# zhoujoey/ORB-SLAM3-Mac

Hardware: AMD Instinct MI355X
Metric: ORB extract+match frames/sec (higher is better)
Workload: dtype u8; 1 GPU; vga: synthetic 640x480 batch=1024 per GPU, 8-level pyramid, 1000 feats/frame, ORB extract + Hamming 2-NN match (Frame.cc:1146) + SearchForInitialization (ORBmatcher.cc:710) vs successor frame; pipelines=1, matchers=side by side (two contexts), frames_total=1024

## Files before the change

### include/orbhip.h

```cpp
#ifndef ORBHIP_H
#define ORBHIP_H
#include <stddef.h>
#include <stdint.h>
#ifdef __cplusplus
extern "C" {
#endif

#define ORBHIP_OK 0
#define ORBHIP_E_BADARG (-1)
#define ORBHIP_E_NODEVICE (-2)
#define ORBHIP_E_HIP (-3)
#define ORBHIP_E_CAPACITY (-4)
#define ORBHIP_E_ABORTED (-5)
#define ORBHIP_E_NOTSPD (-6)
#define ORBHIP_E_EMPTY (-7)

typedef struct {
    float x, y, size, angle, response;
    int32_t octave, class_id;
} orbhip_keypoint;

typedef struct orbhip_ctx orbhip_ctx;
typedef struct orbhip_extractor orbhip_extractor;

// ... 26 lines not shown
int orbhip_extractor_results(orbhip_extractor *ext, orbhip_keypoint **d_kp, uint8_t **d_desc,
                             int32_t **d_count, int32_t **d_mono_index);
int orbhip_extract_batch_host(orbhip_extractor *ext, const uint8_t *h_images, int width, int height,
                              size_t row_stride, size_t frame_stride, int batch, int lap0, int lap1,
                              orbhip_keypoint *kp_out, uint8_t *desc_out, int cap,
                              int32_t *count_out, int32_t *mono_out);
int orbhip_extract_batch_host_view(orbhip_extractor *ext, const uint8_t *h_images, int width, int height, size_t row_stride,
                                   size_t frame_stride, int batch, int lap0, int lap1, const orbhip_keypoint **kp_view,
                                   const uint8_t **desc_view, int *row_capacity, const int32_t **count_view, const int32_t **mono_view);
int orbhip_extractor_blur_kernel(const orbhip_extractor *ext, int batch);
int orbhip_extractor_fast_kernel(const orbhip_extractor *ext);
int orbhip_extractor_blur_tiled(const orbhip_extractor *ext, int batch);
int orbhip_extractor_desc_plan(const orbhip_extractor *ext, int batch, int32_t *kp_base, int32_t *kp_cap, int32_t *waves_per_xcd);

int orbhip_extractor_resize_band_rows(const orbhip_extractor *ext, int level);

int orbhip_extractor_last_frame(orbhip_extractor *ext, int frame, const orbhip_keypoint **d_kp, const uint8_t **d_desc,
                                const orbhip_keypoint **h_kp_view, const uint8_t **h_desc_view, int32_t *count, unsigned long long *generation);

int orbhip_extractor_level_dims(const orbhip_extractor *ext, int level, int *w, int *h);
int orbhip_extractor_get_pyramid_level(orbhip_extractor *ext, int frame, int level, int padded,
                                       uint8_t *h_out, size_t out_stride);
int orbhip_extractor_get_pyramid_padded(orbhip_extractor *ext, int frame, uint8_t *const *levels_out, const size_t *strides);
int orbhip_extractor_get_blurred_level(orbhip_extractor *ext, int frame, int level,
                                       uint8_t *h_out, size_t out_stride);
int orbhip_extractor_get_fast_candidates(orbhip_extractor *ext, int frame, int level,
                                         int32_t *xs, int32_t *ys, int32_t *scores, int cap,
                                         int32_t *n_out);
int orbhip_extractor_get_level_keypoints(orbhip_extractor *ext, int frame, int level,
                                         orbhip_keypoint *out, int cap, int32_t *n_out);
// ... 612 lines not shown
```

### orb-slam3-mac_amd/csrc/orb_internal.h

```cpp
#pragma once
#include <hip/hip_runtime.h>
#include <stdint.h>
#include <vector>
#include "../../include/orbhip.h"

#define ORB_MAX_LEVELS 16
#define ORB_EDGE 19
#define ORB_MINB 16
#define ORB_HALF_PATCH 15
#define ORB_RS_STEPS 24

struct OrbLevel {
    uint8_t *img;
    uint8_t *blur;
    size_t img_frame_stride;
    size_t blur_frame_stride;
    int w, h, img_pitch, blur_pitch;
    int blur_tiles_x;
    int ncols, nrows, wcell, hcell;
    int cell_base;
    int cell_cap;
    int quota;
    int key_base, key_cap;
    int kp_base, kp_cap;
// ... 102 lines not shown
    const int32_t *nL, *nR;
    float mb, mbf;
    float *u_right, *depth;
    int32_t *sad, *n_kept;
};
void orb_launch_stereo(const StereoArgs &A, hipStream_t s);

int orb_lds_optin(const void *func, int device, size_t need);

void orb_plan_fast(const OrbParams &P, FastParams &F);
bool orb_plan_resize(OrbParams &P, int level, const std::vector<int16_t> &xofs, const std::vector<int16_t> &xalpha, const std::vector<int16_t> &yofs,
                     const std::vector<int16_t> &ybeta, std::vector<uint32_t> &xchunk, std::vector<uint32_t> &ytab);
bool orb_plan_blur(OrbParams &P, std::vector<int8_t> &bm_th, std::vector<int8_t> &bm_tv);
int orb_blur_kernel(const OrbParams &P, int batch);

void orb_launch_resize(const OrbParams &P, int level, hipStream_t s);
void orb_launch_fast_cells(const FastParams &F, hipStream_t s, int max_per_cu, int lvl_lo = 0, int lvl_hi = -1);
const void *orb_fast_runs_func(int nld);
int orb_fast_runs_nld(const FastParams &F);
int orb_fast_variant(const FastParams &F);
const void *orb_fast_cells_func(int small);
#define ORB_OVERLAP_MIN_BATCH 16
#ifndef BLR_R
#define BLR_R 24
#endif
void orb_launch_blur(const OrbParams &P, hipStream_t s, int wgs_per_cu, int frame0 = 0, int nframes = -1);
void orb_launch_orient_desc(const OrbParams &P, hipStream_t s);
int orb_orient_desc_blocks(const OrbParams &P);
void orb_launch_octree(const OrbParams &P, hipStream_t s, int parts = 3);
void orb_launch_assemble(const OrbParams &P, hipStream_t s);
size_t orb_octree_lds_bytes(int nc);
// ... 4 lines not shown
```

### orb-slam3-mac_amd/csrc/orbhip_api.hip

```cpp
#include "orb_internal.h"
#include "ctx_internal.h"
#include <cmath>
#include <cfloat>
#include <cstdio>
#include <cstdlib>
#include <cstring>
#include <string>
#include <vector>
#include <mutex>
#include <set>
#include <utility>

static thread_local std::string g_last_error;
extern "C" const char *orbhip_last_error(void) { return g_last_error.c_str(); }
extern "C" const char *orbhip_version(void) { return "orbhip 0.1 (gfx950)"; }

#define HIP_TRY(expr)                                                                   \
    do {                                                                                \
        hipError_t _e = (expr);                                                         \
        if (_e != hipSuccess) {                                                         \
            g_last_error = std::string(#expr) + ": " + hipGetErrorString(_e);           \
            return ORBHIP_E_HIP;                                                        \
        }                                                                               \
    } while (0)
// ... 189 lines not shown
static inline int align_up(int v, int a) { return (v + a - 1) / a * a; }

#define ORBHIP_PROF_SLOTS 32
struct orbhip_extractor {
    orbhip_ctx *ctx;
    int nfeatures, nlevels, ini_th, min_th;
    float scale_factor;
    float scale[ORB_MAX_LEVELS], inv_scale[ORB_MAX_LEVELS], sigma2[ORB_MAX_LEVELS], inv_sigma2[ORB_MAX_LEVELS];
    int per_level[ORB_MAX_LEVELS];
    int umax[ORB_HALF_PATCH + 1];
    int gauss_q8[7];
    int width, height, max_batch;
    bool level0_owned;
    OrbParams P;
    FastParams F;
    std::vector<void *> allocs;
    size_t bytes_reserved;
    int last_batch;
    bool profiling;
    hipEvent_t ev[ORBHIP_PROF_SLOTS][ORBHIP_STAGE_COUNT + 1];
    int ev_calls;
    bool ev_created;
    float stage_ms[ORBHIP_STAGE_COUNT];
    uint8_t *d_level0;
    int32_t *d_stereo_sad;
    bool graph_mode, graph_valid;
    hipStream_t aux; hipEvent_t ev_fork, ev_join, ev_pyr; bool aux_ok; int overlap;
    hipGraphExec_t graph_exec;
    int g_w, g_h, g_batch, g_lap0, g_lap1;
    size_t level0_frame_stride; int level0_pitch;
// ... 96 lines not shown
extern "C" int orbhip_extractor_max_keypoints(const orbhip_extractor *e) { return e ? e->P.max_kp : ORBHIP_E_BADARG; }

template <typename T>
static int dev_alloc(orbhip_extractor *e, T **p, size_t count)
{
    void *q = nullptr;
    size_t bytes = std::max<size_t>(count * sizeof(T), 256);
    hipError_t err = hipMalloc(&q, bytes);
    if (err != hipSuccess) { g_last_error = std::string("hipMalloc: ") + hipGetErrorString(err); return ORBHIP_E_HIP; }
    e->allocs.push_back(q);
    e->bytes_reserved += bytes;
    *p = (T *)q;
    return ORBHIP_OK;
}

static void resize_tables(int sn, int dn, bool horizontal, std::vector<int16_t> &ofs, std::vector<int16_t> &coef)
{
    double scale = 1. / ((double)dn / sn);
    ofs.resize(dn); coef.resize(2 * dn);
    for (int d = 0; d < dn; d++) {
        float f = (float)((d + 0.5) * scale - 0.5);
        int s = (int)floorf(f);
        f -= s;
        if (horizontal) {
            if (s < 0) { f = 0; s = 0; }
            if (s >= sn - 1) { f = 0; s = sn - 1; }
        }
        int c0 = cv_round_f((1.f - f) * 2048), c1 = cv_round_f(f * 2048);
        ofs[d] = (int16_t)std::min(std::max(s, -32768), 32767);
        coef[2 * d] = (int16_t)std::min(std::max(c0, -32768), 32767);
        coef[2 * d + 1] = (int16_t)std::min(std::max(c1, -32768), 32767);
    }
}

extern "C" int orbhip_blur_half_widths(int *out19)
{
    if (!out19) return ORBHIP_E_BADARG;
    static const int8_t pat[1024] = {
#include "orb_pattern.inc"
    };
    double R2 = 0;
    for (int i = 0; i < 512; i++) R2 = std::max(R2, (double)pat[2 * i] * pat[2 * i] + (double)pat[2 * i + 1] * pat[2 * i + 1]);
    for (int d = 0; d < ORB_EDGE; d++) {
        const double t = std::max(d - 0.5, 0.0), q = R2 - t * t;
        out19[d] = q > 0 ? std::min((int)floor(sqrt(q) + 0.5), 18) : -64;
    }
    return ORBHIP_OK;
}

// ... 35 lines not shown
        OrbLevel &L = P.lv[l];
        L.cell_cap = max_cell_cap;
        L.key_base = keys;
        L.key_cap = std::min(L.ncols * L.nrows * max_cell_cap, ((L.w - 2 * ORB_MINB + 1) / 2 + L.ncols) * ((L.h - 2 * ORB_MINB + 1) / 2 + L.nrows));
        L.key_cap = std::min(L.key_cap, 0xFFFFF);
        keys += align_up(L.key_cap, 4);
    }
    P.cells_per_frame = cells; P.keys_per_frame = keys; P.kps_per_frame = kps; P.max_kp = align_up(kps, 8);
    orb_plan_fast(P, e->F);
    P.rows_min_batch = getenv("ORBHIP_ROWS_MIN_BATCH") ? atoi(getenv("ORBHIP_ROWS_MIN_BATCH")) : 16;
    std::vector<int8_t> bm_th, bm_tv;
    const bool bm_ok = orb_plan_blur(P, bm_th, bm_tv);
    P.cell_list_frame_stride = (size_t)cells * max_cell_cap;
    int rc;
    const size_t B = (size_t)max_batch;
    for (int l = 0; l < e->nlevels; l++) {
        OrbLevel &L = P.lv[l];
        L.img_pitch = align_up(L.w, 64); L.blur_pitch = L.img_pitch;
        L.img_frame_stride = (size_t)L.img_pitch * L.h;
        L.blur_tiles_x = (L.w + 15) / 16;
        L.blur_frame_stride = align_up(std::max((size_t)L.blur_pitch * L.h, (size_t)L.blur_tiles_x * ((L.h + 7) / 8) * 128), (size_t)128);
        if ((rc = dev_alloc(e, &L.img, B * L.img_frame_stride + 64))) return rc;
        if ((rc = dev_alloc(e, &L.blur, B * L.blur_frame_stride + 64))) return rc;
        if (l > 0) {
            std::vector<int16_t> xo, xa, yo, yb;
            resize_tables(P.lv[l - 1].w, L.w, true, xo, xa);
            resize_tables(P.lv[l - 1].h, L.h, false, yo, yb);
            int16_t *dxo, *dxa, *dyo, *dyb;
            if ((rc = dev_alloc(e, &dxo, xo.size()))) return rc;
            if ((rc = dev_alloc(e, &dxa, xa.size()))) return rc;
            if ((rc = dev_alloc(e, &dyo, yo.size()))) return rc;
            if ((rc = dev_alloc(e, &dyb, yb.size()))) return rc;
            HIP_TRY(hipMemcpy(dxo, xo.data(), xo.size() * 2, hipMemcpyHostToDevice));
            HIP_TRY(hipMemcpy(dxa, xa.data(), xa.size() * 2, hipMemcpyHostToDevice));
            HIP_TRY(hipMemcpy(dyo, yo.data(), yo.size() * 2, hipMemcpyHostToDevice));
            HIP_TRY(hipMemcpy(dyb, yb.data(), yb.size() * 2, hipMemcpyHostToDevice));
            L.xofs = dxo; L.xalpha = dxa; L.yofs = dyo; L.ybeta = dyb;
            L.xchunk = nullptr; L.ytab = nullptr;
            std::vector<uint32_t> xc, yt;
            if (orb_plan_resize(P, l, xo, xa, yo, yb, xc, yt)) {
                uint32_t *dxc, *dyt;
                if ((rc = dev_alloc(e, &dxc, xc.size()))) return rc;
                if ((rc = dev_alloc(e, &dyt, yt.size()))) return rc;
                HIP_TRY(hipMemcpy(dxc, xc.data(), xc.size() * 4, hipMemcpyHostToDevice));
                HIP_TRY(hipMemcpy(dyt, yt.data(), yt.size() * 4, hipMemcpyHostToDevice));
                L.xchunk = dxc; L.ytab = dyt;
            }
        }
    }
    e->d_level0 = P.lv[0].img; e->level0_pitch = P.lv[0].img_pitch; e->level0_frame_stride = P.lv[0].img_frame_stride;
    if (bm_ok) {
        uint4 *dth, *dtv;
        if ((rc = dev_alloc(e, &dth, bm_th.size() / 16))) return rc;
        if ((rc = dev_alloc(e, &dtv, bm_tv.size() / 16))) return rc;
        HIP_TRY(hipMemcpy(dth, bm_th.data(), bm_th.size(), hipMemcpyHostToDevice));
        HIP_TRY(hipMemcpy(dtv, bm_tv.data(), bm_tv.size(), hipMemcpyHostToDevice));
        P.bm_th = dth; P.bm_tv = dtv;
    }
    P.desc_blocks_cap = getenv("ORBHIP_TUNE_DESC_BLOCKS") ? atoi(getenv("ORBHIP_TUNE_DESC_BLOCKS")) : 0;
    orbhip_blur_half_widths(P.blur_hw);
    if ((rc = dev_alloc(e, &P.cell_count, B * cells))) return rc;
// ... 181 lines not shown
    return orb_fast_variant(e->F);
}

extern "C" int orbhip_extractor_blur_tiled(const orbhip_extractor *e, int batch)
{
    if (!e || !e->max_batch) return -1;
    return e->P.blur_tiled_ok && orb_blur_kernel(e->P, batch) == 2 ? 1 : 0;
}

extern "C" int orbhip_extractor_resize_band_rows(const orbhip_extractor *e, int level)
{
    if (!e || !e->max_batch || level < 1 || level >= e->nlevels) return -1;
    return e->P.lv[level].xchunk ? e->P.lv[level].rs_rows : 0;
}

extern "C" int orbhip_extractor_set_profiling(orbhip_extractor *e, int enable)
{
    if (!e) return ORBHIP_E_BADARG;
    if (enable && !e->ev_created) {
        for (auto &slot : e->ev) for (auto &ev : slot) HIP_TRY(hipEventCreate(&ev));
        e->ev_created = true;
    }
    e->profiling = enable != 0;
    e->ev_calls = 0;
    return ORBHIP_OK;
}

extern "C" int orbhip_extractor_stage_ms(orbhip_extractor *e, float *ms_out)
{
    if (!e || !ms_out || !e->ev_created || e->ev_calls <= 0) return ORBHIP_E_BADARG;
// ... 29 lines not shown
        HIP_TRY(hipEventCreateWithFlags(&e->ev_fork, hipEventDisableTiming));
        HIP_TRY(hipEventCreateWithFlags(&e->ev_join, hipEventDisableTiming));
        HIP_TRY(hipEventCreateWithFlags(&e->ev_pyr, hipEventDisableTiming));
        e->aux_ok = true;
    }
    FastParams &F = e->F;
    for (int l = 0; l < e->nlevels; l++) { F.lv[l].img = P.lv[l].img; F.lv[l].frame_stride = P.lv[l].img_frame_stride; F.lv[l].img_pitch = P.lv[l].img_pitch; }
    F.batch = batch; F.n_cus = e->ctx->n_cus; F.cell_count = P.cell_count; F.cell_list = P.cell_list; F.cell_list_frame_stride = P.cell_list_frame_stride; F.status = P.status;
    const bool rows = orb_blur_kernel(P, batch) != 0;
    const int fast_waves = fork ? tune_int("ORBHIP_TUNE_FAST_WAVES", rows ? 18 : 10) : 0;
    STAGE_MARK(ORBHIP_STAGE_PYRAMID);
    if (fork && e->nlevels > 1 && rows && tune_int("ORBHIP_TUNE_L0_EARLY", 0)) {
        HIP_TRY(hipEventRecord(e->ev_fork, s));
        HIP_TRY(hipStreamWaitEvent(e->aux, e->ev_fork, 0));
        orb_launch_fast_cells(F, s, fast_waves, 0, 1);
        for (int l = 1; l < e->nlevels; l++) orb_launch_resize(P, l, e->aux);
        HIP_TRY(hipEventRecord(e->ev_pyr, e->aux));
        HIP_TRY(hipStreamWaitEvent(s, e->ev_pyr, 0));
        orb_launch_fast_cells(F, s, fast_waves, 1, e->nlevels);
        orb_launch_blur(P, e->aux, 5);
        HIP_TRY(hipEventRecord(e->ev_join, e->aux));
    } else {
        for (int l = 1; l < e->nlevels; l++) orb_launch_resize(P, l, s);
        STAGE_MARK(ORBHIP_STAGE_FAST_CELLS);
        if (fork) {
            HIP_TRY(hipEventRecord(e->ev_fork, s));
            HIP_TRY(hipStreamWaitEvent(e->aux, e->ev_fork, 0));
        }
        orb_launch_fast_cells(F, s, fast_waves);
        if (fork) {
            if (!tune_int("ORBHIP_TUNE_SKIP_BLUR", 0))
                orb_launch_blur(P, e->aux, tune_int("ORBHIP_TUNE_BLUR_WGS", 5));
            HIP_TRY(hipEventRecord(e->ev_join, e->aux));
        }
    }
    STAGE_MARK(ORBHIP_STAGE_BLUR);
    if (!fork) orb_launch_blur(P, s, 8);
    STAGE_MARK(ORBHIP_STAGE_OCTREE);
// ... 385 lines not shown
```

### orb-slam3-mac_amd/csrc/pyramid_kernels.hip

```cpp
#include "orb_internal.h"
#include "wave_dpp.h"
#include <algorithm>
#include <cstdlib>

#define RS_TW 64
#define RS_TH 32
#define RS_MAXC 144
#define RS_MAXR 68
__global__ __launch_bounds__(256) void k_resize(OrbParams P, int level)
{
    __shared__ __attribute__((aligned(16))) uint32_t in[RS_MAXR * (RS_MAXC / 4)];
    __shared__ uint16_t hz[RS_MAXR * RS_TW];
    const OrbLevel &D = P.lv[level];
    const OrbLevel &S = P.lv[level - 1];
    const int tid = threadIdx.x;
    const int ntx = (D.w + RS_TW - 1) / RS_TW, nty = (D.h + RS_TH - 1) / RS_TH;
    const unsigned lid = xcd_logical_id(blockIdx.x, gridDim.x);
    const int frame = lid / (ntx * nty), trem = lid - frame * (ntx * nty);
    const int dx0 = (trem % ntx) * RS_TW, dy0 = (trem / ntx) * RS_TH;
    const int dx_last = min(dx0 + RS_TW, D.w) - 1, dy_last = min(dy0 + RS_TH, D.h) - 1;
    const int ybase = D.yofs[dy0];
    const int nrows = min(D.yofs[dy_last] + 1 - ybase + 1, RS_MAXR);
    const int xbase = D.xofs[dx0] & ~15;
    const int nc16 = min((D.xofs[dx_last] + 1 - xbase) / 16 + 1, RS_MAXC / 16);
// ... 140 lines not shown
                const uint32_t s0 = rs_mulhi24(t.z, h0) + rs_mulhi24(t.w, n0) + 2u;
                const uint32_t s1 = rs_mulhi24(t.z, h1) + rs_mulhi24(t.w, n1) + 2u;
                const uint32_t s2 = rs_mulhi24(t.z, h2) + rs_mulhi24(t.w, n2) + 2u;
                const uint32_t s3 = rs_mulhi24(t.z, h3) + rs_mulhi24(t.w, n3) + 2u;
                const uint32_t p01 = (s0 | (s1 << 16)) >> 2, p23 = (s2 | (s3 << 16)) >> 2;
                if (t.y) {
                    *reinterpret_cast<uint32_t *>(dst + doff) = __builtin_amdgcn_perm(p23, p01, 0x06040200u);
                    doff += (uint32_t)D.img_pitch;
                }
            }
            h0 = n0; h1 = n1; h2 = n2; h3 = n3;
        }
    }
}

bool orb_plan_resize(OrbParams &P, int level, const std::vector<int16_t> &xo, const std::vector<int16_t> &xa, const std::vector<int16_t> &yo,
                     const std::vector<int16_t> &yb, std::vector<uint32_t> &xc, std::vector<uint32_t> &yt)
{
    OrbLevel &L = P.lv[level];
    const int l = level, sw = P.lv[l - 1].w, sh = P.lv[l - 1].h, nch = (L.w + 3) / 4;
    xc.assign((size_t)nch * 12, 0); yt.clear();
    bool fits = sw >= 8 && nch >= 4;
    const char *rm = getenv("ORBHIP_RESIZE_MODE");
    int mode = l > 1 || (sw % 4 == 0 && sw >= 12) ? 1 : 0;
    if (rm && atoi(rm) == 0) mode = 0;
    for (int c = 0; c < nch && fits; c++) {
        const int base = std::min((int)xo[4 * c], sw - 8);
        const int base4 = l > 1 ? (base & ~3) : std::min(base & ~3, sw - 12);
        xc[12 * c] = mode ? (uint32_t)base4 : (uint32_t)base;
        xc[12 * c + 9] = 0x03020100u + 0x01010101u * (uint32_t)(base - base4);
        for (int j = 0; j < 4; j++) {
            const int col = std::min(4 * c + j, L.w - 1);
            const int i0 = xo[col] - base, a0 = xa[2 * col], a1 = xa[2 * col + 1];
            int i1 = i0 + 1;
            if (i0 < 0 || i0 > 7 || a0 < 0 || a1 < 0) { fits = false; break; }
            if (i1 > 7) { if (a1 != 0) { fits = false; break; } i1 = i0; }
            xc[12 * c + 1 + j] = (uint32_t)i0 | 0x0c00u | ((uint32_t)i1 << 16) | 0x0c000000u;
            xc[12 * c + 5 + j] = (uint32_t)a0 | ((uint32_t)a1 << 16);
        }
    }
    for (int dy = 0; dy < L.h; dy++)
        if (yb[2 * dy] < 0 || yb[2 * dy + 1] < 0 || yb[2 * dy] > 2048 || yb[2 * dy + 1] > 2048) fits = false;
    auto band_steps = [&](int y0, int y1, std::vector<uint32_t> *out) {
        int n = 0, prev = -1;
        for (int dy = y0; dy < y1; dy++) {
            const int r0 = std::min(std::max((int)yo[dy], 0), sh - 1), r1 = std::min(std::max((int)yo[dy] + 1, 0), sh - 1);
            if (n == 0 || prev != r0) {
                if (out) { const uint32_t e[4] = {(uint32_t)r0, 0u, 0u, 0u}; out->insert(out->end(), e, e + 4); }
                n++;
            }
            if (out) { const uint32_t e[4] = {(uint32_t)r1, 1u, (uint32_t)yb[2 * dy] << 12, (uint32_t)yb[2 * dy + 1] << 12}; out->insert(out->end(), e, e + 4); }
            n++; prev = r1;
        }
        return n;
    };
    int rsr = ORB_RS_STEPS - 1;
    for (; rsr > 1; rsr--) {
        bool ok = true;
        for (int y0 = 0; y0 < L.h && ok; y0 += rsr) ok = band_steps(y0, std::min(y0 + rsr, L.h), nullptr) <= ORB_RS_STEPS;
        if (ok) break;
    }
    L.rs_rows = rsr;
    for (int y0 = 0; y0 < L.h && fits; y0 += rsr) {
        const size_t at = yt.size();
        band_steps(y0, std::min(y0 + rsr, L.h), &yt);
        while (yt.size() < at + 4 * ORB_RS_STEPS) {
            const uint32_t e[4] = {yt[yt.size() - 4], 0u, 0u, 0u};
            yt.insert(yt.end(), e, e + 4);
        }
    }
// ... 4 lines not shown

void orb_launch_resize(const OrbParams &P, int level, hipStream_t s)
{
    const OrbLevel &D = P.lv[level];
    if (D.xchunk && P.batch >= P.rows_min_batch) {
        const int nch = (D.w + 3) >> 2, nb = (D.h + D.rs_rows - 1) / D.rs_rows, nbx = (nch * nb + 255) / 256;
        const dim3 grid((unsigned)nbx * (unsigned)P.batch);
        const size_t lds = (size_t)((256 / nch + 2) * RS_STEPS) * sizeof(uint4);
        if (D.resize_mode == 1) hipLaunchKernelGGL(k_resize_rows<1>, grid, dim3(256), lds, s, P, level, nbx);
        else hipLaunchKernelGGL(k_resize_rows<0>, grid, dim3(256), lds, s, P, level, nbx);
        return;
    }
    const unsigned nblocks = (unsigned)(((D.w + RS_TW - 1) / RS_TW) * ((D.h + RS_TH - 1) / RS_TH)) * (unsigned)P.batch;
    hipLaunchKernelGGL(k_resize, dim3(nblocks), dim3(256), 0, s, P, level);
}
```

### orb-slam3-mac_amd/python/orbhip.py

```python
import ctypes as C
import os
import numpy as np

try:
    import torch
except Exception:
    torch = None

_HERE = os.path.dirname(os.path.abspath(__file__))
LIB_DIR = os.path.join(os.path.dirname(_HERE), "lib")
LIB_PATH = os.path.join(LIB_DIR, "liborbhip.so")
SYNTH_PATH = os.path.join(LIB_DIR, "libsynth.so")

if not os.path.exists(LIB_PATH):
    raise ImportError(
        "liborbhip.so not built: run `python -c 'import __graft_entry__ as g; g.build()'` "
        "(there is no CPU fallback for the HIP path)")

lib = C.CDLL(LIB_PATH)

OK, E_BADARG, E_NODEVICE, E_HIP, E_CAPACITY, E_ABORTED, E_NOTSPD, E_EMPTY = 0, -1, -2, -3, -4, -5, -6, -7
STAGES = ["pyramid", "fast_cells", "blur", "octree", "desc", "assemble"]

KP_DTYPE = np.dtype([("x", "<f4"), ("y", "<f4"), ("size", "<f4"), ("angle", "<f4"),
# ... 32 lines not shown
lib.orbhip_descriptor_distance.argtypes = [vp, vp]
lib.orbhip_match_bf2nn_device.argtypes = [vp, vp, vp, sz, vp, vp, sz, ci, ci, cd, vp, vp, vp]
lib.orbhip_search_for_initialization_device.argtypes = [vp, vp, vp, vp, vp, vp, vp, ci, ci, sz, cf, cf, cf, cf, ci, cf, ci,
                                                        vp, vp, vp]
lib.orbhip_ctx_check_status.argtypes = [vp]
lib.orbhip_ctx_wait_for.argtypes = [vp, vp]
lib.orbhip_extractor_blur_kernel.argtypes = [vp, ci]
lib.orbhip_extractor_blur_kernel.restype = ci
if hasattr(lib, "orbhip_extractor_fast_kernel"):
    lib.orbhip_extractor_fast_kernel.argtypes = [vp]
    lib.orbhip_extractor_fast_kernel.restype = ci
lib.orbhip_extractor_blur_tiled.argtypes = [vp, ci]
lib.orbhip_extractor_blur_tiled.restype = ci
lib.orbhip_extractor_resize_band_rows.argtypes = [vp, ci]
lib.orbhip_extractor_resize_band_rows.restype = ci
if hasattr(lib, "orbhip_extractor_desc_plan"):
    lib.orbhip_extractor_desc_plan.argtypes = [vp, ci, vp, vp, C.POINTER(ci)]
if hasattr(lib, "orbhip_debug_octree"):
    lib.orbhip_debug_octree.argtypes = [vp, ci, ci, vp, vp, vp, vp, ci, vp, ci, vp, vp]
lib.orbhip_prev_matched_init_device.argtypes = [vp, vp, sz, ci, ci, vp]
lib.orbhip_search_by_projection_device.argtypes = [vp, vp, vp, vp, ci, vp, vp, vp, vp, ci, sz, ci, cf, cf, cf, cf, ci, ci, vp, vp]
lib.orbhip_search_local_map_device.argtypes = [vp, vp, vp, vp, ci, vp, vp, vp, vp, ci, sz, ci, cf, cf, cf, cf, ci, cf, vp, vp]


class OrbHipError(RuntimeError):
    def __init__(self, code, where):
        self.code = code
        super().__init__("%s failed: %d (%s)" % (where, code, lib.orbhip_last_error().decode()))


# ... 21 lines not shown
    def stream(self):
        return lib.orbhip_ctx_stream(self.h)

    def close(self):
        if self.h:
            lib.orbhip_ctx_destroy(self.h)
            self.h = None


def blur_half_widths():
    out = np.zeros(19, np.int32)
    _chk(lib.orbhip_blur_half_widths(out.ctypes.data), "orbhip_blur_half_widths")
    return out


class Extractor:

    def __init__(self, ctx, nfeatures=1000, scale_factor=1.2, nlevels=8, ini_th=20, min_th=7):
        h = vp()
        _chk(lib.orbhip_extractor_create(ctx.h, nfeatures, scale_factor, nlevels, ini_th, min_th, C.byref(h)),
             "orbhip_extractor_create")
        self.h, self.ctx, self.nlevels = h, ctx, nlevels

    def close(self):
        if self.h:
            lib.orbhip_extractor_destroy(self.h)
            self.h = None

    def table(self, which):
        out = np.zeros(self.nlevels, np.float32)
# ... 21 lines not shown
        return ("k_blur", "k_blur_rows", "k_blur_mfma")[lib.orbhip_extractor_blur_kernel(self.h, int(batch))]

    def fast_kernel(self):
        return lib.orbhip_extractor_fast_kernel(self.h)

    def blur_tiled(self, batch):
        return lib.orbhip_extractor_blur_tiled(self.h, int(batch)) == 1

    def desc_plan(self, batch):
        base, cap, waves = np.zeros(self.nlevels, np.int32), np.zeros(self.nlevels, np.int32), ci()
        _chk(lib.orbhip_extractor_desc_plan(self.h, int(batch), base.ctypes.data, cap.ctypes.data, C.byref(waves)), "desc_plan")
        return base, cap, waves.value

    def resize_band_rows(self, level):
        return lib.orbhip_extractor_resize_band_rows(self.h, int(level))

    def debug_octree(self, level, lists, form):
        offs = np.zeros(len(lists) + 1, np.int32)
        offs[1:] = np.cumsum([len(l[0]) for l in lists])
        xs, ys, ss = (np.ascontiguousarray(np.concatenate([np.asarray(l[k], np.int32) for l in lists] + [np.zeros(1, np.int32)])) for k in range(3))
        cap = int(max(len(l[0]) for l in lists)) + 16
        keys = np.zeros((len(lists), cap), np.uint32)
        counts, redo = np.zeros(len(lists), np.int32), np.zeros(len(lists), np.int32)
        _chk(lib.orbhip_debug_octree(self.h, int(level), len(lists), offs.ctypes.data, xs.ctypes.data, ys.ctypes.data, ss.ctypes.data,
                                     {"iterative": 0, "table": 1}[form], keys.ctypes.data, cap, counts.ctypes.data, redo.ctypes.data),
             "orbhip_debug_octree")
        kept = [np.stack([k & 0xFFF, (k >> 12) & 0xFFF, k >> 24], 1).astype(np.int32) for k in (keys[f, :counts[f]] for f in range(len(lists)))]
        return kept, redo.tolist()

    def set_graph_mode(self, on):
# ... 1195 lines not shown
```

Baseline: 347,700 frames/s.

## Fuse pairs of pyramid resize levels into one kernel via LDS intermediate

Adds a grouped resize kernel that computes two consecutive pyramid levels per tile. The intermediate level is kept in shared memory (LDS) and the second downscale reads from it instead of global memory. A host planner builds per-group tile, halo and step tables, and launches fall back to single-level resizes when grouping fails or the batch is small. This cuts kernel launches and global re-reads of intermediate levels, at the cost of halo recomputation, LDS pressure and lower occupancy.

```diff
diff --git a/include/orbhip.h b/include/orbhip.h
--- a/include/orbhip.h
+++ b/include/orbhip.h
@@ -64,6 +64,10 @@
 int orbhip_extractor_desc_plan(const orbhip_extractor *ext, int batch, int32_t *kp_base, int32_t *kp_cap, int32_t *waves_per_xcd);
 
 int orbhip_extractor_resize_band_rows(const orbhip_extractor *ext, int level);
+
+int orbhip_extractor_resize_groups(const orbhip_extractor *ext, int *sizes, int cap);
+
+int orbhip_pyramid_group_plan(int width, int height, float scale_factor, int nlevels, int max_group, int32_t *out, int cap);
 
 int orbhip_extractor_last_frame(orbhip_extractor *ext, int frame, const orbhip_keypoint **d_kp, const uint8_t **d_desc,
                                 const orbhip_keypoint **h_kp_view, const uint8_t **h_desc_view, int32_t *count, unsigned long long *generation);
diff --git a/orb-slam3-mac_amd/csrc/orb_internal.h b/orb-slam3-mac_amd/csrc/orb_internal.h
--- a/orb-slam3-mac_amd/csrc/orb_internal.h
+++ b/orb-slam3-mac_amd/csrc/orb_internal.h
@@ -140,7 +140,36 @@
 bool orb_plan_blur(OrbParams &P, std::vector<int8_t> &bm_th, std::vector<int8_t> &bm_tv);
 int orb_blur_kernel(const OrbParams &P, int batch);
 
+#define ORB_RG_MAXN 2
+#define ORB_RG_LDS_CAP (40 * 1024)
+struct RgLevel { uint8_t *img; size_t frame_stride; int pitch; const uint32_t *xc; };
+struct ResizeGroupArgs {
+    RgLevel lv[ORB_RG_MAXN + 1];
+    int ntx, nty;
+    int nsub[ORB_RG_MAXN];
+    int sbase[ORB_RG_MAXN + 1];
+    int rbase[ORB_RG_MAXN];
+    int rpitch[ORB_RG_MAXN];
+    const int4 *tx;
+    const int4 *ty;
+    const uint4 *steps;
+};
+struct OrbResizeTabs { std::vector<int16_t> xo, xa, yo, yb; bool rows; int mode; };
+struct OrbResizeGroup {
+    int first, n;
+    int tw, th;
+    int mode;
+    int lanes0;
+    size_t lds_bytes;
+    std::vector<int32_t> tx, ty;
+    std::vector<uint32_t> steps, xc[ORB_RG_MAXN];
+    ResizeGroupArgs args;
+};
+void orb_resize_tables(int sn, int dn, bool horizontal, std::vector<int16_t> &ofs, std::vector<int16_t> &coef);
+void orb_plan_resize_groups(int nlevels, const int *w, const int *h, const std::vector<OrbResizeTabs> &T, int max_group, std::vector<OrbResizeGroup> &out);
+
 void orb_launch_resize(const OrbParams &P, int level, hipStream_t s);
+void orb_launch_pyramid(const OrbParams &P, std::vector<OrbResizeGroup> &groups, hipStream_t s);
 void orb_launch_fast_cells(const FastParams &F, hipStream_t s, int max_per_cu, int lvl_lo = 0, int lvl_hi = -1);
 const void *orb_fast_runs_func(int nld);
 int orb_fast_runs_nld(const FastParams &F);
diff --git a/orb-slam3-mac_amd/csrc/orbhip_api.hip b/orb-slam3-mac_amd/csrc/orbhip_api.hip
--- a/orb-slam3-mac_amd/csrc/orbhip_api.hip
+++ b/orb-slam3-mac_amd/csrc/orbhip_api.hip
@@ -227,6 +227,7 @@
     bool level0_owned;
     OrbParams P;
     FastParams F;
+    std::vector<OrbResizeGroup> pyr;
     std::vector<void *> allocs;
     size_t bytes_reserved;
     int last_batch;
@@ -353,25 +354,6 @@
     return ORBHIP_OK;
 }
 
-static void resize_tables(int sn, int dn, bool horizontal, std::vector<int16_t> &ofs, std::vector<int16_t> &coef)
-{
-    double scale = 1. / ((double)dn / sn);
-    ofs.resize(dn); coef.resize(2 * dn);
-    for (int d = 0; d < dn; d++) {
-        float f = (float)((d + 0.5) * scale - 0.5);
-        int s = (int)floorf(f);
-        f -= s;
-        if (horizontal) {
-            if (s < 0) { f = 0; s = 0; }
-            if (s >= sn - 1) { f = 0; s = sn - 1; }
-        }
-        int c0 = cv_round_f((1.f - f) * 2048), c1 = cv_round_f(f * 2048);
-        ofs[d] = (int16_t)std::min(std::max(s, -32768), 32767);
-        coef[2 * d] = (int16_t)std::min(std::max(c0, -32768), 32767);
-        coef[2 * d + 1] = (int16_t)std::min(std::max(c1, -32768), 32767);
-    }
-}
-
 extern "C" int orbhip_blur_half_widths(int *out19)
 {
     if (!out19) return ORBHIP_E_BADARG;
@@ -437,6 +419,7 @@
     P.cell_list_frame_stride = (size_t)cells * max_cell_cap;
     int rc;
     const size_t B = (size_t)max_batch;
+    std::vector<OrbResizeTabs> rtabs(e->nlevels);
     for (int l = 0; l < e->nlevels; l++) {
         OrbLevel &L = P.lv[l];
         L.img_pitch = align_up(L.w, 64); L.blur_pitch = L.img_pitch;
@@ -446,9 +429,9 @@
         if ((rc = dev_alloc(e, &L.img, B * L.img_frame_stride + 64))) return rc;
         if ((rc = dev_alloc(e, &L.blur, B * L.blur_frame_stride + 64))) return rc;
         if (l > 0) {
-            std::vector<int16_t> xo, xa, yo, yb;
-            resize_tables(P.lv[l - 1].w, L.w, true, xo, xa);
-            resize_tables(P.lv[l - 1].h, L.h, false, yo, yb);
+            std::vector<int16_t> &xo = rtabs[l].xo, &xa = rtabs[l].xa, &yo = rtabs[l].yo, &yb = rtabs[l].yb;
+            orb_resize_tables(P.lv[l - 1].w, L.w, true, xo, xa);
+            orb_resize_tables(P.lv[l - 1].h, L.h, false, yo, yb);
             int16_t *dxo, *dxa, *dyo, *dyb;
             if ((rc = dev_alloc(e, &dxo, xo.size()))) return rc;
             if ((rc = dev_alloc(e, &dxa, xa.size()))) return rc;
@@ -468,6 +451,30 @@
                 HIP_TRY(hipMemcpy(dxc, xc.data(), xc.size() * 4, hipMemcpyHostToDevice));
                 HIP_TRY(hipMemcpy(dyt, yt.data(), yt.size() * 4, hipMemcpyHostToDevice));
                 L.xchunk = dxc; L.ytab = dyt;
+            }
+            rtabs[l].rows = L.xchunk != nullptr; rtabs[l].mode = L.resize_mode;
+        }
+    }
+    {
+        int lw[ORB_MAX_LEVELS], lh[ORB_MAX_LEVELS];
+        for (int l = 0; l < e->nlevels; l++) { lw[l] = P.lv[l].w; lh[l] = P.lv[l].h; }
+        const int max_group = getenv("ORBHIP_RESIZE_GROUP") ? atoi(getenv("ORBHIP_RESIZE_GROUP")) : 2;
+        orb_plan_resize_groups(e->nlevels, lw, lh, rtabs, max_group, e->pyr);
+        for (OrbResizeGroup &g : e->pyr) {
+            if (g.n == 1) continue;
+            int32_t *dtx, *dty; uint32_t *dst;
+            if ((rc = dev_alloc(e, &dtx, g.tx.size()))) return rc;
+            if ((rc = dev_alloc(e, &dty, g.ty.size()))) return rc;
+            if ((rc = dev_alloc(e, &dst, g.steps.size()))) return rc;
+            HIP_TRY(hipMemcpy(dtx, g.tx.data(), g.tx.size() * 4, hipMemcpyHostToDevice));
+            HIP_TRY(hipMemcpy(dty, g.ty.data(), g.ty.size() * 4, hipMemcpyHostToDevice));
+            HIP_TRY(hipMemcpy(dst, g.steps.data(), g.steps.size() * 4, hipMemcpyHostToDevice));
+            g.args.tx = reinterpret_cast<const int4 *>(dtx); g.args.ty = reinterpret_cast<const int4 *>(dty); g.args.steps = reinterpret_cast<const uint4 *>(dst);
+            for (int k = 1; k < g.n; k++) {
+                uint32_t *dxc;
+                if ((rc = dev_alloc(e, &dxc, g.xc[k].size()))) return rc;
+                HIP_TRY(hipMemcpy(dxc, g.xc[k].data(), g.xc[k].size() * 4, hipMemcpyHostToDevice));
+                g.args.lv[k + 1].xc = dxc;
             }
         }
     }
@@ -679,6 +686,13 @@
     return e->P.lv[level].xchunk ? e->P.lv[level].rs_rows : 0;
 }
 
+extern "C" int orbhip_extractor_resize_groups(const orbhip_extractor *e, int *sizes, int cap)
+{
+    if (!e || !e->max_batch) return -1;
+    for (size_t i = 0; i < e->pyr.size() && (int)i < cap && sizes; i++) sizes[i] = e->pyr[i].n;
+    return (int)e->pyr.size();
+}
+
 extern "C" int orbhip_extractor_set_profiling(orbhip_extractor *e, int enable)
 {
     if (!e) return ORBHIP_E_BADARG;
@@ -738,14 +752,14 @@
         HIP_TRY(hipEventRecord(e->ev_fork, s));
         HIP_TRY(hipStreamWaitEvent(e->aux, e->ev_fork, 0));
         orb_launch_fast_cells(F, s, fast_waves, 0, 1);
-        for (int l = 1; l < e->nlevels; l++) orb_launch_resize(P, l, e->aux);
+        orb_launch_pyramid(P, e->pyr, e->aux);
         HIP_TRY(hipEventRecord(e->ev_pyr, e->aux));
         HIP_TRY(hipStreamWaitEvent(s, e->ev_pyr, 0));
         orb_launch_fast_cells(F, s, fast_waves, 1, e->nlevels);
         orb_launch_blur(P, e->aux, 5);
         HIP_TRY(hipEventRecord(e->ev_join, e->aux));
     } else {
-        for (int l = 1; l < e->nlevels; l++) orb_launch_resize(P, l, s);
+        orb_launch_pyramid(P, e->pyr, s);
         STAGE_MARK(ORBHIP_STAGE_FAST_CELLS);
         if (fork) {
             HIP_TRY(hipEventRecord(e->ev_fork, s));
diff --git a/orb-slam3-mac_amd/csrc/pyramid_kernels.hip b/orb-slam3-mac_amd/csrc/pyramid_kernels.hip
--- a/orb-slam3-mac_amd/csrc/pyramid_kernels.hip
+++ b/orb-slam3-mac_amd/csrc/pyramid_kernels.hip
@@ -1,7 +1,9 @@
 #include "orb_internal.h"
 #include "wave_dpp.h"
 #include <algorithm>
+#include <cmath>
 #include <cstdlib>
+#include <cstring>
 
 #define RS_TW 64
 #define RS_TH 32
@@ -178,6 +180,92 @@
     }
 }
 
+template <int MODE, bool SRC_LDS, bool DST_LDS>
+__device__ __forceinline__ void rg_stage(const uint8_t *src, uint32_t spitch, uint32_t srow0, uint32_t scol0, const uint32_t *xctab, int4 X, int4 Y,
+                                         int nsub, const uint4 *st, uint8_t *dst, uint32_t dpitch, uint8_t *ldst, uint32_t lpitch)
+{
+    const unsigned g = threadIdx.x, nch = (unsigned)X.y;
+    if (g >= nch * (unsigned)nsub) return;
+    const unsigned sub = g / nch, cl = g - sub * nch, c = (unsigned)X.x + cl;
+    const bool own = (int)c >= X.z && (int)c < X.w;
+    const uint4 *xc = reinterpret_cast<const uint4 *>(xctab) + 3 * c;
+    const uint4 x0 = xc[0], x1 = xc[1];
+    const uint4 x2 = xc[2];
+    const uint32_t al3 = x2.x, shsel = x2.y;
+    const uint32_t base = x0.x - scol0, sel0 = x0.y, sel1 = x0.z, sel2 = x0.w, sel3 = x1.x, al0 = x1.y, al1 = x1.z, al2 = x1.w;
+    st += sub * RS_STEPS;
+    uint2 q[2][8];
+#pragma unroll
+    for (int u = 0; u < 8; u++) q[0][u] = rs_load8<MODE>(src, __umul24(st[u].x - srow0, spitch) + base, shsel);
+    const uint32_t row0 = st[0].z;
+    uint32_t doff = __umul24(row0, dpitch) + 4 * c, loff = __umul24(row0 - (uint32_t)Y.x, lpitch) + 4 * cl;
+    uint32_t h0 = 0, h1 = 0, h2 = 0, h3 = 0;
+#pragma unroll
+    for (int g = 0; g < RS_STEPS / 8; g++) {
+        if (g + 1 < RS_STEPS / 8) {
+#pragma unroll
+            for (int u = 0; u < 8; u++) q[(g + 1) & 1][u] = rs_load8<MODE>(src, __umul24(st[8 * (g + 1) + u].x - srow0, spitch) + base, shsel);
+        }
+#pragma unroll
+        for (int u = 0; u < 8; u++) {
+            const uint2 a = q[g & 1][u];
+            const uint32_t n0 = rs_hpass(a, sel0, al0), n1 = rs_hpass(a, sel1, al1), n2 = rs_hpass(a, sel2, al2), n3 = rs_hpass(a, sel3, al3);
+            if (8 * g + u > 0) {
+                const uint4 t = st[8 * g + u];
+                const uint32_t s0 = rs_mulhi24(t.z, h0) + rs_mulhi24(t.w, n0) + 2u;
+                const uint32_t s1 = rs_mulhi24(t.z, h1) + rs_mulhi24(t.w, n1) + 2u;
+                const uint32_t s2 = rs_mulhi24(t.z, h2) + rs_mulhi24(t.w, n2) + 2u;
+                const uint32_t s3 = rs_mulhi24(t.z, h3) + rs_mulhi24(t.w, n3) + 2u;
+                const uint32_t p01 = (s0 | (s1 << 16)) >> 2, p23 = (s2 | (s3 << 16)) >> 2;
+                if (t.y) {
+                    const uint32_t px = __builtin_amdgcn_perm(p23, p01, 0x06040200u);
+                    if (DST_LDS) { *reinterpret_cast<uint32_t *>(ldst + loff) = px; loff += lpitch; }
+                    if ((t.y & 2u) && own) *reinterpret_cast<uint32_t *>(dst + doff) = px;
+                    doff += dpitch;
+                }
+            }
+            h0 = n0; h1 = n1; h2 = n2; h3 = n3;
+        }
+    }
+}
+template <int MODE>
+__global__ __launch_bounds__(256) void k_resize_group(ResizeGroupArgs G)
+{
+    extern __shared__ uint4 gl[];
+    const unsigned tiles = (unsigned)(G.ntx * G.nty);
+    const unsigned lid = xcd_logical_id(blockIdx.x, gridDim.x);
+    const unsigned frame = lid / tiles, t = lid - frame * tiles;
+    const unsigned ty = t / (unsigned)G.ntx, tx = t - ty * (unsigned)G.ntx;
+    const int nst = G.sbase[2];
+    for (int i = (int)threadIdx.x; i < nst; i += 256) gl[i] = G.steps[ty * (unsigned)nst + i];
+    uint8_t *rect = reinterpret_cast<uint8_t *>(gl + nst);
+    __syncthreads();
+    const int4 XA = G.tx[tx * 2], YA = G.ty[ty * 2];
+    rg_stage<MODE, false, true>(G.lv[0].img + (size_t)frame * G.lv[0].frame_stride, (uint32_t)G.lv[0].pitch, 0u, 0u, G.lv[1].xc, XA, YA, G.nsub[0],
+                                gl + G.sbase[0], G.lv[1].img + (size_t)frame * G.lv[1].frame_stride, (uint32_t)G.lv[1].pitch, rect, (uint32_t)G.rpitch[0]);
+    __syncthreads();
+    rg_stage<1, true, false>(rect, (uint32_t)G.rpitch[0], (uint32_t)YA.x, 4u * (uint32_t)XA.x, G.lv[2].xc, G.tx[tx * 2 + 1], G.ty[ty * 2 + 1], G.nsub[1],
+                             gl + G.sbase[1], G.lv[2].img + (size_t)frame * G.lv[2].frame_stride, (uint32_t)G.lv[2].pitch, nullptr, 0u);
+}
+
+static int rs_band_steps(const std::vector<int16_t> &yo, const std::vector<int16_t> &yb, int sh, int y0, int y1, int own0, int own1, std::vector<uint32_t> *out)
+{
+    int n = 0, prev = -1;
+    for (int dy = y0; dy < y1; dy++) {
+        const int r0 = std::min(std::max((int)yo[dy], 0), sh - 1), r1 = std::min(std::max((int)yo[dy] + 1, 0), sh - 1);
+        if (n == 0 || prev != r0) {
+            if (out) { const uint32_t e[4] = {(uint32_t)r0, 0u, 0u, 0u}; out->insert(out->end(), e, e + 4); }
+            n++;
+        }
+        if (out) {
+            const uint32_t e[4] = {(uint32_t)r1, dy >= own0 && dy < own1 ? 3u : 1u, (uint32_t)yb[2 * dy] << 12, (uint32_t)yb[2 * dy + 1] << 12};
+            out->insert(out->end(), e, e + 4);
+        }
+        n++; prev = r1;
+    }
+    return n;
+}
+
 bool orb_plan_resize(OrbParams &P, int level, const std::vector<int16_t> &xo, const std::vector<int16_t> &xa, const std::vector<int16_t> &yo,
                      const std::vector<int16_t> &yb, std::vector<uint32_t> &xc, std::vector<uint32_t> &yt)
 {
@@ -205,19 +293,7 @@
     }
     for (int dy = 0; dy < L.h; dy++)
         if (yb[2 * dy] < 0 || yb[2 * dy + 1] < 0 || yb[2 * dy] > 2048 || yb[2 * dy + 1] > 2048) fits = false;
-    auto band_steps = [&](int y0, int y1, std::vector<uint32_t> *out) {
-        int n = 0, prev = -1;
-        for (int dy = y0; dy < y1; dy++) {
-            const int r0 = std::min(std::max((int)yo[dy], 0), sh - 1), r1 = std::min(std::max((int)yo[dy] + 1, 0), sh - 1);
-            if (n == 0 || prev != r0) {
-                if (out) { const uint32_t e[4] = {(uint32_t)r0, 0u, 0u, 0u}; out->insert(out->end(), e, e + 4); }
-                n++;
-            }
-            if (out) { const uint32_t e[4] = {(uint32_t)r1, 1u, (uint32_t)yb[2 * dy] << 12, (uint32_t)yb[2 * dy + 1] << 12}; out->insert(out->end(), e, e + 4); }
-            n++; prev = r1;
-        }
-        return n;
-    };
+    auto band_steps = [&](int y0, int y1, std::vector<uint32_t> *out) { return rs_band_steps(yo, yb, sh, y0, y1, 0, 0, out); };
     int rsr = ORB_RS_STEPS - 1;
     for (; rsr > 1; rsr--) {
         bool ok = true;
@@ -252,3 +328,265 @@
     const unsigned nblocks = (unsigned)(((D.w + RS_TW - 1) / RS_TW) * ((D.h + RS_TH - 1) / RS_TH)) * (unsigned)P.batch;
     hipLaunchKernelGGL(k_resize, dim3(nblocks), dim3(256), 0, s, P, level);
 }
+
+void orb_resize_tables(int sn, int dn, bool horizontal, std::vector<int16_t> &ofs, std::vector<int16_t> &coef)
+{
+    double scale = 1. / ((double)dn / sn);
+    ofs.resize(dn); coef.resize(2 * dn);
+    for (int d = 0; d < dn; d++) {
+        float f = (float)((d + 0.5) * scale - 0.5);
+        int s = (int)floorf(f);
+        f -= s;
+        if (horizontal) {
+            if (s < 0) { f = 0; s = 0; }
+            if (s >= sn - 1) { f = 0; s = sn - 1; }
+        }
+        int c0 = (int)lrintf((1.f - f) * 2048), c1 = (int)lrintf(f * 2048);
+        ofs[d] = (int16_t)std::min(std::max(s, -32768), 32767);
+        coef[2 * d] = (int16_t)std::min(std::max(c0, -32768), 32767);
+        coef[2 * d + 1] = (int16_t)std::min(std::max(c1, -32768), 32767);
+    }
+}
+
+static int rg_window(const std::vector<int16_t> &xo, int c, int sw, int *base_out)
+{
+    const int base = std::min((int)xo[4 * c], sw - 8);
+    if (base_out) *base_out = base;
+    return std::min(base & ~3, ((sw + 3) & ~3) - 12);
+}
+
+namespace {
+struct RgSide {
+    bool ok; int nt, maxn[ORB_RG_MAXN], nsub[ORB_RG_MAXN]; long sum0;
+    std::vector<int32_t> tab;
+    std::vector<std::vector<uint32_t>> steps;
+};
+}
+static void rg_side_x(int first, int n, const int *w, const std::vector<OrbResizeTabs> &T, int tw, RgSide &S)
+{
+    const int deep = first + n - 1, nchd = (w[deep] + 3) / 4;
+    S.ok = true; S.nt = (nchd + tw - 1) / tw; S.tab.assign((size_t)S.nt * n * 4, 0); S.sum0 = 0;
+    for (int k = 0; k < n; k++) S.maxn[k] = 0;
+    for (int t = 0; t < S.nt; t++) {
+        int c0 = t * tw, c1 = std::min(c0 + tw, nchd);
+        for (int k = n - 1; k >= 0; k--) {
+            int32_t *e = &S.tab[((size_t)t * n + k) * 4];
+            e[0] = c0; e[1] = c1 - c0;
+            S.maxn[k] = std::max(S.maxn[k], c1 - c0);
+            if (k == 0) { S.sum0 += c1 - c0; break; }
+            const int sw = w[first + k - 1], nchs = (sw + 3) / 4;
+            int lo = nchs, hi = 0;
+            for (int c = c0; c < c1; c++) { const int b4 = rg_window(T[first + k].xo, c, sw, nullptr); lo = std::min(lo, b4 / 4); hi = std::max(hi, b4 / 4 + 3); }
+            if (t == 0) lo = 0;
+            if (t == S.nt - 1) hi = nchs;
+            if (lo < 0 || hi > nchs) S.ok = false;
+            c0 = lo; c1 = hi;
+        }
+    }
+    for (int t = 0; t < S.nt && S.ok; t++)
+        for (int k = 0; k < n; k++) {
+            int32_t *e = &S.tab[((size_t)t * n + k) * 4];
+            e[2] = e[0];
+            e[3] = k == n - 1 || t == S.nt - 1 ? e[0] + e[1] : S.tab[((size_t)(t + 1) * n + k) * 4];
+            if (e[3] <= e[2] || e[3] > e[0] + e[1]) S.ok = false;
+        }
+}
+static void rg_side_y(int first, int n, const int *h, const std::vector<OrbResizeTabs> &T, int th, bool tables, RgSide &S)
+{
+    const int deep = first + n - 1, hd = h[deep];
+    S.ok = true; S.nt = (hd + th - 1) / th; S.tab.assign((size_t)S.nt * n * 4, 0); S.sum0 = 0;
+    for (int k = 0; k < n; k++) S.maxn[k] = S.nsub[k] = 0;
+    for (int t = 0; t < S.nt; t++) {
+        int y0 = t * th, y1 = std::min(y0 + th, hd);
+        for (int k = n - 1; k >= 0; k--) {
+            int32_t *e = &S.tab[((size_t)t * n + k) * 4];
+            e[0] = y0; e[1] = y1 - y0;
+            S.maxn[k] = std::max(S.maxn[k], y1 - y0);
+            if (k == 0) { S.sum0 += y1 - y0; break; }
+            const int sh = h[first + k - 1];
+            const std::vector<int16_t> &yo = T[first + k].yo;
+            int lo = sh, hi = 0;
+            for (int y = y0; y < y1; y++) {
+                lo = std::min(lo, std::min(std::max((int)yo[y], 0), sh - 1));
+                hi = std::max(hi, std::min(std::max((int)yo[y] + 1, 0), sh - 1) + 1);
+            }
+            if (t == 0) lo = 0;
+            if (t == S.nt - 1) hi = sh;
+            y0 = lo; y1 = hi;
+        }
+    }
+    for (int t = 0; t < S.nt && S.ok; t++)
+        for (int k = 0; k < n; k++) {
+            int32_t *e = &S.tab[((size_t)t * n + k) * 4];
+            e[2] = e[0];
+            e[3] = k == n - 1 || t == S.nt - 1 ? e[0] + e[1] : S.tab[((size_t)(t + 1) * n + k) * 4];
+            if (e[3] <= e[2] || e[3] > e[0] + e[1]) S.ok = false;
+        }
+    if (!S.ok) return;
+    if (tables) S.steps.assign((size_t)S.nt * n, std::vector<uint32_t>());
+    for (int t = 0; t < S.nt; t++)
+        for (int k = 0; k < n; k++) {
+            const int32_t *e = &S.tab[((size_t)t * n + k) * 4];
+            const OrbResizeTabs &L = T[first + k];
+            const int sh = h[first + k - 1];
+            int nsub = 0;
+            for (int y0 = e[0]; y0 < e[0] + e[1]; nsub++) {
+                int y1 = y0 + 1;
+                while (y1 < e[0] + e[1] && rs_band_steps(L.yo, L.yb, sh, y0, y1 + 1, 0, 0, nullptr) <= ORB_RS_STEPS) y1++;
+                if (tables) {
+                    std::vector<uint32_t> &o = S.steps[(size_t)t * n + k];
+                    const size_t at = o.size();
+                    rs_band_steps(L.yo, L.yb, sh, y0, y1, e[2], e[3], &o);
+                    o[at + 2] = (uint32_t)y0;
+                    while (o.size() < at + 4 * ORB_RS_STEPS) { const uint32_t p[4] = {o[o.size() - 4], 0u, 0u, 0u}; o.insert(o.end(), p, p + 4); }
+                }
+                y0 = y1;
+            }
+            S.nsub[k] = std::max(S.nsub[k], nsub);
+        }
+}
+static bool rg_plan_group(int first, int n, const int *w, const int *h, const std::vector<OrbResizeTabs> &T, OrbResizeGroup &g)
+{
+    const int deep = first + n - 1, nchd = (w[deep] + 3) / 4, hd = h[deep];
+    std::vector<RgSide> XS, YS;
+    std::vector<int> tws, ths;
+    for (int tw = 4; tw <= std::min(nchd, 64); tw++) { RgSide S; rg_side_x(first, n, w, T, tw, S); if (S.ok) { XS.push_back(S); tws.push_back(tw); } }
+    for (int th = 4; th <= std::min(hd, 256); th++) { RgSide S; rg_side_y(first, n, h, T, th, false, S); if (S.ok) { YS.push_back(S); ths.push_back(th); } }
+    long best_wg = -1, best_area = 0; size_t bx = 0, by = 0;
+    for (size_t i = 0; i < XS.size(); i++)
+        for (size_t j = 0; j < YS.size(); j++) {
+            const RgSide &X = XS[i], &Y = YS[j];
+            bool ok = true; size_t lds = 0;
+            for (int k = 0; k < n; k++) {
+                ok = ok && X.maxn[k] * Y.nsub[k] <= 256;
+                lds += (size_t)Y.nsub[k] * ORB_RS_STEPS * 16;
+                if (k < n - 1) lds += (size_t)Y.maxn[k] * 4 * X.maxn[k];
+            }
+            if (!ok || lds > ORB_RG_LDS_CAP) continue;
+            const long wg = (long)X.nt * Y.nt, area = X.sum0 * Y.sum0;
+            if (best_wg < 0 || wg < best_wg || (wg == best_wg && area < best_area)) { best_wg = wg; best_area = area; bx = i; by = j; }
+        }
+    if (best_wg < 0) return false;
+    const RgSide &X = XS[bx];
+    RgSide Y; rg_side_y(first, n, h, T, ths[by], true, Y);
+    g = OrbResizeGroup();
+    g.first = first; g.n = n; g.tw = tws[bx]; g.th = ths[by]; g.mode = T[first].mode;
+    g.tx = X.tab; g.ty = Y.tab;
+    ResizeGroupArgs &A = g.args;
+    memset(&A, 0, sizeof(A));
+    A.ntx = X.nt; A.nty = Y.nt;
+    size_t lds = 0;
+    for (int k = 0; k < n; k++) { A.nsub[k] = Y.nsub[k]; A.sbase[k] = k ? A.sbase[k - 1] + Y.nsub[k - 1] * ORB_RS_STEPS : 0; }
+    A.sbase[n] = A.sbase[n - 1] + Y.nsub[n - 1] * ORB_RS_STEPS;
+    lds = (size_t)A.sbase[n] * 16;
+    for (int k = 0; k < n - 1; k++) { A.rbase[k] = (int)(lds - (size_t)A.sbase[n] * 16); A.rpitch[k] = 4 * X.maxn[k]; lds += (size_t)Y.maxn[k] * A.rpitch[k]; }
+    g.lds_bytes = lds;
+    g.steps.clear();
+    for (int t = 0; t < Y.nt; t++)
+        for (int k = 0; k < n; k++) {
+            std::vector<uint32_t> o = Y.steps[(size_t)t * n + k];
+            while (o.size() < (size_t)4 * ORB_RS_STEPS * Y.nsub[k]) { const uint32_t p[4] = {o[o.size() - 4], 0u, (uint32_t)g.ty[((size_t)t * n + k) * 4], 0u}; o.insert(o.end(), p, p + 4); }
+            g.steps.insert(g.steps.end(), o.begin(), o.end());
+        }
+    for (int k = 1; k < n; k++) {
+        const OrbResizeTabs &L = T[first + k];
+        const int sw = w[first + k - 1], lw = w[first + k], nch = (lw + 3) / 4;
+        std::vector<uint32_t> &xc = g.xc[k];
+        xc.assign((size_t)nch * 12, 0);
+        for (int c = 0; c < nch; c++) {
+            int base; const int base4 = rg_window(L.xo, c, sw, &base);
+            xc[12 * c] = (uint32_t)base4;
+            xc[12 * c + 9] = 0x03020100u + 0x01010101u * (uint32_t)(base - base4);
+            for (int j = 0; j < 4; j++) {
+                const int col = std::min(4 * c + j, lw - 1);
+                const int i0 = L.xo[col] - base;
+                const int i1 = i0 + 1 > 7 ? i0 : i0 + 1;
+                xc[12 * c + 1 + j] = (uint32_t)i0 | 0x0c00u | ((uint32_t)i1 << 16) | 0x0c000000u;
+                xc[12 * c + 5 + j] = (uint32_t)L.xa[2 * col] | ((uint32_t)L.xa[2 * col + 1] << 16);
+            }
+        }
+    }
+    long lanes = 0;
+    for (int tx = 0; tx < X.nt; tx++)
+        for (int ty = 0; ty < Y.nt; ty++) {
+            int nsub = 0;
+            for (int y0 = 0; y0 < (int)Y.steps[(size_t)ty * n].size(); y0 += 4 * ORB_RS_STEPS) nsub++;
+            lanes += (long)X.tab[((size_t)tx * n) * 4 + 1] * nsub;
+        }
+    g.lanes0 = (int)(lanes / ((long)X.nt * Y.nt));
+    return true;
+}
+
+void orb_plan_resize_groups(int nlevels, const int *w, const int *h, const std::vector<OrbResizeTabs> &T, int max_group, std::vector<OrbResizeGroup> &out)
+{
+    out.clear();
+    max_group = std::min(std::max(max_group, 1), ORB_RG_MAXN);
+    for (int l = 1; l < nlevels;) {
+        int n = 1;
+        if (T[l].rows) while (n < max_group && l + n < nlevels && T[l + n].rows) n++;
+        OrbResizeGroup g;
+        while (n > 1 && !rg_plan_group(l, n, w, h, T, g)) n--;
+        if (n == 1) { g = OrbResizeGroup(); g.first = l; g.n = 1; memset(&g.args, 0, sizeof(g.args)); }
+        out.push_back(g);
+        l += n;
+    }
+}
+
+extern "C" int orbhip_pyramid_group_plan(int width, int height, float scale_factor, int nlevels, int max_group, int32_t *out, int cap)
+{
+    if (width <= 0 || height <= 0 || nlevels < 1 || nlevels > ORB_MAX_LEVELS || !(scale_factor > 1.0f) || scale_factor > 2.0f) return -1;
+    static OrbParams P;
+    memset(&P, 0, sizeof(P));
+    int w[ORB_MAX_LEVELS], h[ORB_MAX_LEVELS];
+    float s = 1.0f;
+    for (int l = 0; l < nlevels; l++) {
+        if (l) s *= scale_factor;
+        const float inv = 1.0f / s;
+        w[l] = P.lv[l].w = (int)lrintf((float)width * inv); h[l] = P.lv[l].h = (int)lrintf((float)height * inv);
+        if (w[l] < 2 || h[l] < 2) return -1;
+    }
+    std::vector<OrbResizeTabs> T(nlevels);
+    for (int l = 1; l < nlevels; l++) {
+        orb_resize_tables(w[l - 1], w[l], true, T[l].xo, T[l].xa);
+        orb_resize_tables(h[l - 1], h[l], false, T[l].yo, T[l].yb);
+        std::vector<uint32_t> xc, yt;
+        T[l].rows = orb_plan_resize(P, l, T[l].xo, T[l].xa, T[l].yo, T[l].yb, xc, yt);
+        T[l].mode = P.lv[l].resize_mode;
+    }
+    std::vector<OrbResizeGroup> G;
+    orb_plan_resize_groups(nlevels, w, h, T, max_group, G);
+    std::vector<int32_t> o;
+    o.push_back((int32_t)G.size());
+    for (const OrbResizeGroup &g : G) {
+        const ResizeGroupArgs &A = g.args;
+        const int32_t hd[8] = {g.first, g.n, g.tw, g.th, A.ntx, A.nty, (int32_t)g.lds_bytes, g.lanes0};
+        o.insert(o.end(), hd, hd + 8);
+        o.insert(o.end(), A.nsub, A.nsub + ORB_RG_MAXN); o.insert(o.end(), A.sbase, A.sbase + ORB_RG_MAXN + 1); o.insert(o.end(), A.rbase, A.rbase + ORB_RG_MAXN);
+        o.insert(o.end(), A.rpitch, A.rpitch + ORB_RG_MAXN);
+        if (g.n == 1) continue;
+        o.insert(o.end(), g.tx.begin(), g.tx.end()); o.insert(o.end(), g.ty.begin(), g.ty.end());
+        o.insert(o.end(), g.steps.begin(), g.steps.end());
+        for (int k = 1; k < g.n; k++) o.insert(o.end(), g.xc[k].begin(), g.xc[k].end());
+    }
+    for (size_t i = 0; i < o.size() && (long)i < (long)cap && out; i++) out[i] = o[i];
+    return (int)o.size();
+}
+
+void orb_launch_pyramid(const OrbParams &P, std::vector<OrbResizeGroup> &groups, hipStream_t s)
+{
+    for (OrbResizeGroup &g : groups) {
+        if (g.n == 1 || P.batch < P.rows_min_batch) {
+            for (int l = g.first; l < g.first + g.n; l++) orb_launch_resize(P, l, s);
+            continue;
+        }
+        ResizeGroupArgs &A = g.args;
+        for (int k = 0; k <= g.n; k++) {
+            const OrbLevel &L = P.lv[g.first - 1 + k];
+            A.lv[k].img = L.img; A.lv[k].frame_stride = L.img_frame_stride; A.lv[k].pitch = L.img_pitch;
+        }
+        A.lv[1].xc = P.lv[g.first].xchunk;
+        const dim3 grid((unsigned)(A.ntx * A.nty) * (unsigned)P.batch);
+        if (g.mode == 1) hipLaunchKernelGGL(k_resize_group<1>, grid, dim3(256), g.lds_bytes, s, A);
+        else hipLaunchKernelGGL(k_resize_group<0>, grid, dim3(256), g.lds_bytes, s, A);
+    }
+}
diff --git a/orb-slam3-mac_amd/host/host_pyramid_plan_sweep.cc b/orb-slam3-mac_amd/host/host_pyramid_plan_sweep.cc
--- /dev/null
+++ b/orb-slam3-mac_amd/host/host_pyramid_plan_sweep.cc
@@ -0,0 +1,34 @@
+#include <cstdint>
+#include <cstdio>
+#include <vector>
+
+extern "C" int orbhip_pyramid_group_plan(int width, int height, float scale_factor, int nlevels, int max_group, int32_t *out, int cap);
+
+static long g_plans = 0, g_words = 0;
+
+static int one(int w, int h, float scale, int nlev, int max_group)
+{
+    const int need = orbhip_pyramid_group_plan(w, h, scale, nlev, max_group, nullptr, 0);
+    if (need < 0) return 0;
+    std::vector<int32_t> buf((size_t)need);
+    if (orbhip_pyramid_group_plan(w, h, scale, nlev, max_group, buf.data(), need) != need) { fprintf(stderr, "size changed: %d x %d\n", w, h); return 1; }
+    if (buf[0] < 1 || buf[0] > nlev - 1) { fprintf(stderr, "group count %d: %d x %d\n", buf[0], w, h); return 1; }
+    g_plans++; g_words += need;
+    return 0;
+}
+
+int main()
+{
+    const float scales[3] = {1.1f, 1.2f, 1.44f};
+    const int levels[3] = {5, 8, 12}, heights[2] = {240, 277};
+    int bad = 0;
+    for (float s : scales)
+        for (int nl : levels) {
+            for (int w = 320; w <= 400; w++)
+                for (int h : heights)
+                    for (int mg = 1; mg <= 2; mg++) bad += one(w, h, s, nl, mg);
+            bad += one(640, 480, s, nl, 2) + one(1920, 1080, s, nl, 2) + one(3840, 2160, s, nl, 2);
+        }
+    printf("%ld plans, %ld words, %d bad\n", g_plans, g_words, bad);
+    return bad ? 1 : 0;
+}
diff --git a/orb-slam3-mac_amd/python/orbhip.py b/orb-slam3-mac_amd/python/orbhip.py
--- a/orb-slam3-mac_amd/python/orbhip.py
+++ b/orb-slam3-mac_amd/python/orbhip.py
@@ -70,6 +70,11 @@
 lib.orbhip_extractor_blur_tiled.restype = ci
 lib.orbhip_extractor_resize_band_rows.argtypes = [vp, ci]
 lib.orbhip_extractor_resize_band_rows.restype = ci
+if hasattr(lib, "orbhip_extractor_resize_groups"):
+    lib.orbhip_extractor_resize_groups.argtypes = [vp, vp, ci]
+    lib.orbhip_extractor_resize_groups.restype = ci
+    lib.orbhip_pyramid_group_plan.argtypes = [ci, ci, C.c_float, ci, ci, vp, ci]
+    lib.orbhip_pyramid_group_plan.restype = ci
 if hasattr(lib, "orbhip_extractor_desc_plan"):
     lib.orbhip_extractor_desc_plan.argtypes = [vp, ci, vp, vp, C.POINTER(ci)]
 if hasattr(lib, "orbhip_debug_octree"):
@@ -121,6 +126,43 @@
     return out
 
 
+def pyramid_level_sizes(width, height, scale_factor, nlevels):
+    s, out = np.float32(1.0), []
+    for l in range(nlevels):
+        if l:
+            s = np.float32(s * np.float32(scale_factor))
+        inv = np.float32(1.0) / s
+        out.append((int(np.rint(np.float32(width) * inv)), int(np.rint(np.float32(height) * inv))))
+    return out
+
+
+def pyramid_group_plan(width, height, scale_factor, nlevels, max_group=2):
+    args = (int(width), int(height), float(scale_factor), int(nlevels), int(max_group))
+    need = lib.orbhip_pyramid_group_plan(*args, None, 0)
+    if need < 0:
+        raise OrbHipError("pyramid_group_plan: bad geometry")
+    buf = np.zeros(need, np.int32)
+    lib.orbhip_pyramid_group_plan(*args, buf.ctypes.data, need)
+    sizes = pyramid_level_sizes(width, height, scale_factor, nlevels)
+    groups, at = [], [1]
+
+    def take(*shape):
+        a = buf[at[0]:at[0] + int(np.prod(shape))].reshape(shape)
+        at[0] += a.size
+        return a
+    for _ in range(int(buf[0])):
+        g = dict(zip(("first", "n", "tw", "th", "ntx", "nty", "lds_bytes", "lanes0"), (int(v) for v in take(8))))
+        g["nsub"], g["sbase"], g["rbase"], g["rpitch"] = take(2), take(3), take(2), take(2)
+        n = g["n"]
+        if n > 1:
+            g["tx"], g["ty"] = take(g["ntx"], n, 4), take(g["nty"], n, 4)
+            g["steps"] = take(g["nty"], int(g["sbase"][n]), 4).view(np.uint32)
+            g["xc"] = {k: take((sizes[g["first"] + k][0] + 3) // 4, 12).view(np.uint32) for k in range(1, n)}
+        groups.append(g)
+    assert at[0] == need
+    return groups
+
+
 class Extractor:
 
     def __init__(self, ctx, nfeatures=1000, scale_factor=1.2, nlevels=8, ini_th=20, min_th=7):
@@ -172,6 +214,11 @@
 
     def resize_band_rows(self, level):
         return lib.orbhip_extractor_resize_band_rows(self.h, int(level))
+
+    def resize_groups(self):
+        sizes = np.zeros(16, np.int32)
+        n = lib.orbhip_extractor_resize_groups(self.h, sizes.ctypes.data, 16)
+        return [int(v) for v in sizes[:max(n, 0)]]
 
     def debug_octree(self, level, lists, form):
         offs = np.zeros(len(lists) + 1, np.int32)
```

New measurement: 349,900 frames/s (median of 6 runs). No clear change (+0.6%).
